# ksil/LFPSQP.jl

Hardware: AMD Instinct MI355X
Metric: projected-CG iters/sec at n=1e7, m=128 fp64 (higher is better)
Workload: dtype f64

## Files before the change

### include/lfpsqp_hip.h

```cpp
#ifndef LFPSQP_HIP_H
#define LFPSQP_HIP_H

#include <stdint.h>

#ifdef __cplusplus
extern "C" {
#endif

#define LFPSQP_OK 0
#define LFPSQP_ERR_ARG (-1)
#define LFPSQP_ERR_HIP (-2)
#define LFPSQP_ERR_COMM (-3)
#define LFPSQP_ERR_NUMERIC (-4)
#define LFPSQP_ERR_UNSUPPORTED (-5)

typedef struct lfpsqp_ctx lfpsqp_ctx;
typedef struct lfpsqp_vec lfpsqp_vec;
typedef struct lfpsqp_mat lfpsqp_mat;
typedef struct lfpsqp_spmat lfpsqp_spmat;

int lfpsqp_ctx_create(int device, lfpsqp_ctx** out);
int lfpsqp_ctx_destroy(lfpsqp_ctx* ctx);
int lfpsqp_ctx_sync(lfpsqp_ctx* ctx);
const char* lfpsqp_last_error(const lfpsqp_ctx* ctx);
int lfpsqp_device_name(const lfpsqp_ctx* ctx, char* buf, int64_t buflen);
int lfpsqp_device_uuid(const lfpsqp_ctx* ctx, char* buf, int64_t buflen);
int lfpsqp_ctx_set_tuning(lfpsqp_ctx* ctx, int ks, int nt);
int lfpsqp_ctx_set_onepass(lfpsqp_ctx* ctx, int mode);
int lfpsqp_ctx_set_residual_buffers(lfpsqp_ctx* ctx, int mode);
int lfpsqp_timer_begin(lfpsqp_ctx* ctx);
int lfpsqp_timer_end(lfpsqp_ctx* ctx, double* ms);

int lfpsqp_shard_range(int64_t n, int rank, int nranks, int64_t* row0, int64_t* row1);
int lfpsqp_comm_unique_id(lfpsqp_ctx* ctx, void* id128);
int lfpsqp_comm_init_rccl(lfpsqp_ctx* ctx, int rank, int nranks, const void* id128);
typedef int (*lfpsqp_allreduce_fn)(void* user, double* buf, int64_t count, int op, void* stream);
int lfpsqp_comm_init_callback(lfpsqp_ctx* ctx, int rank, int nranks, lfpsqp_allreduce_fn fn, void* user);
int lfpsqp_comm_p2p_export(lfpsqp_ctx* ctx, void* handle64);
int lfpsqp_comm_init_p2p(lfpsqp_ctx* ctx, int rank, int nranks, const void* handles);
#define LFPSQP_P2P_MEM_NONE 0
#define LFPSQP_P2P_MEM_FINE 1
#define LFPSQP_P2P_MEM_COARSE 2
int lfpsqp_comm_p2p_allow_coarse(lfpsqp_ctx* ctx, int allow);
int lfpsqp_comm_p2p_info(const lfpsqp_ctx* ctx, int* mem_kind, unsigned long long* collectives);
int lfpsqp_comm_info(const lfpsqp_ctx* ctx, int* rank, int* nranks);

int lfpsqp_vec_alloc(lfpsqp_ctx* ctx, int64_t n, lfpsqp_vec** out);
int lfpsqp_vec_free(lfpsqp_ctx* ctx, lfpsqp_vec* v);
int64_t lfpsqp_vec_len(const lfpsqp_vec* v);
int lfpsqp_vec_upload(lfpsqp_ctx* ctx, lfpsqp_vec* v, int64_t offset, const double* host, int64_t count);
int lfpsqp_vec_download(lfpsqp_ctx* ctx, const lfpsqp_vec* v, int64_t offset, double* host, int64_t count);
int lfpsqp_vec_fill(lfpsqp_ctx* ctx, lfpsqp_vec* v, double value);
int lfpsqp_vec_copy(lfpsqp_ctx* ctx, lfpsqp_vec* dst, const lfpsqp_vec* src);
int lfpsqp_vec_copy_range(lfpsqp_ctx* ctx, lfpsqp_vec* dst, int64_t dst_off, const lfpsqp_vec* src, int64_t src_off, int64_t count);
int lfpsqp_mat_alloc(lfpsqp_ctx* ctx, int64_t n, int64_t m, lfpsqp_mat** out);
int lfpsqp_mat_free(lfpsqp_ctx* ctx, lfpsqp_mat* M);
int lfpsqp_mat_shape(const lfpsqp_mat* M, int64_t* n, int64_t* m);
int lfpsqp_mat_upload(lfpsqp_ctx* ctx, lfpsqp_mat* M, int64_t col0, int64_t ncols, const double* host, int64_t ldh);
int lfpsqp_mat_download(lfpsqp_ctx* ctx, const lfpsqp_mat* M, int64_t col0, int64_t ncols, double* host, int64_t ldh);
int lfpsqp_mat_copy(lfpsqp_ctx* ctx, lfpsqp_mat* dst, const lfpsqp_mat* src);
int lfpsqp_mat_view(lfpsqp_ctx* ctx, const lfpsqp_mat* A, const lfpsqp_vec* rs, const lfpsqp_vec* u, const lfpsqp_vec* w, lfpsqp_mat** out);
int lfpsqp_mat_rowscaled_view(lfpsqp_ctx* ctx, const lfpsqp_mat* A, const lfpsqp_vec* rs, lfpsqp_mat** out);
int lfpsqp_ctx_set_placement(lfpsqp_ctx* ctx, int tries);
int lfpsqp_mat_alloc_placed(lfpsqp_ctx* ctx, int64_t n, int64_t m, lfpsqp_mat** out);
int lfpsqp_vecs_alloc_placed(lfpsqp_ctx* ctx, const lfpsqp_mat* M, int64_t ncols, int64_t n, int count, lfpsqp_vec** out);
int lfpsqp_basis_work_alloc_placed(lfpsqp_ctx* ctx, int64_t n, int64_t m, int64_t nvec, int count, lfpsqp_mat** M_out, lfpsqp_vec** out);
int lfpsqp_placement_info(const lfpsqp_ctx* ctx, int* tries, int* picked, double* ms, int ms_cap);
int lfpsqp_placement_probe(lfpsqp_ctx* ctx, const lfpsqp_mat* M, int64_t ncols, lfpsqp_vec* g, lfpsqp_vec* d, lfpsqp_vec* a, int reps, double* ms);
int lfpsqp_vec_hash_fill(lfpsqp_ctx* ctx, lfpsqp_vec* v, uint64_t seed, int64_t offset, double scale, double shift);
int lfpsqp_mat_hash_fill(lfpsqp_ctx* ctx, lfpsqp_mat* M, uint64_t seed, int64_t row0, int64_t n_global, double scale, int64_t nrows,
                         int64_t ncols);

int lfpsqp_gemv_t(lfpsqp_ctx* ctx, const lfpsqp_mat* M, int64_t ncols, const lfpsqp_vec* v, lfpsqp_vec* t);
int lfpsqp_gemv_n(lfpsqp_ctx* ctx, const lfpsqp_mat* M, int64_t ncols, double alpha, const lfpsqp_vec* t, double beta, lfpsqp_vec* y);
int lfpsqp_dot(lfpsqp_ctx* ctx, const lfpsqp_vec* x, const lfpsqp_vec* y, double* out);
int lfpsqp_dot_head(lfpsqp_ctx* ctx, const lfpsqp_vec* x, const lfpsqp_vec* y, int64_t count, double* out);
int lfpsqp_nrm2(lfpsqp_ctx* ctx, const lfpsqp_vec* x, double* out);
int lfpsqp_amax(lfpsqp_ctx* ctx, const lfpsqp_vec* x, double* out);
int lfpsqp_axpby(lfpsqp_ctx* ctx, double a, const lfpsqp_vec* x, double b, lfpsqp_vec* y);
int lfpsqp_waxpby(lfpsqp_ctx* ctx, double a, const lfpsqp_vec* x, double b, const lfpsqp_vec* y, lfpsqp_vec* z);
int lfpsqp_vmul(lfpsqp_ctx* ctx, const lfpsqp_vec* d, const lfpsqp_vec* x, lfpsqp_vec* y);
int lfpsqp_vec_fill_range(lfpsqp_ctx* ctx, lfpsqp_vec* v, int64_t offset, int64_t count, double value);
// ... 231 lines not shown
```

### lfpsqp.jl_amd/_capi.py

```python
from __future__ import annotations

import ctypes as C
import os
import re

_HERE = os.path.dirname(os.path.abspath(__file__))
DEFAULT_LIB = os.path.join(_HERE, "lib", "liblfpsqp_hip.so")
HEADER = os.path.join(os.path.dirname(_HERE), "include", "lfpsqp_hip.h")

c_i64 = C.c_int64
c_dbl = C.c_double
P = C.c_void_p
PD = C.POINTER(C.c_double)


class DiagOp(C.Structure):
    _fields_ = [("a0", c_dbl), ("dg", P)]


class LowRankOp(C.Structure):
    _fields_ = [("a0", c_dbl), ("dg", P), ("V", P), ("k", c_i64), ("sigma", P)]


class TridiagOp(C.Structure):
    _fields_ = [("a0", c_dbl), ("dg", P), ("off", P)]


class Basis(C.Structure):
    _fields_ = [("Z", P), ("ncols", c_i64), ("Dx", P), ("Dy", P), ("sx", P), ("sy", P), ("A", P), ("W", P), ("S", P), ("SA", P)]


class IneqData(C.Structure):
    _fields_ = [("q", P), ("r", P), ("s", P), ("t", P), ("n", c_i64)]


class Elementwise(C.Structure):
    _fields_ = [("A", P), ("Asp", P), ("kind", P), ("qw", P), ("work", P)]


class Constraints(C.Structure):
    _fields_ = [("Jct", P), ("m_lin", c_i64), ("b", P), ("has_ball", C.c_int), ("R2", c_dbl), ("n_x", c_i64), ("slack_row", c_i64), ("Jsp", P),
                ("ew", C.POINTER(Elementwise))]


CFUN = C.CFUNCTYPE(C.c_int, P, P, PD)
JACFUN = C.CFUNCTYPE(C.c_int, P, P, P, PD)


class PPWork(C.Structure):
    _fields_ = [(k, P) for k in ("r", "p", "z", "dx", "g", "tmp_m", "tmp_w", "h", "DxS", "DyS", "ones", "zeros", "q", "i11", "i12", "i22")] + \
               [("precondition", C.c_int)]


class PcgPrecond(C.Structure):
    _fields_ = [("K", P), ("i11", P), ("i12", P), ("i22", P), ("q", P)]


class ProjCGWorkC(C.Structure):
    _fields_ = [("g", P), ("d", P), ("rp", P), ("Utr", P)]


ALLREDUCE_FN = C.CFUNCTYPE(C.c_int, P, P, c_i64, C.c_int, P)
OPFUN = C.CFUNCTYPE(C.c_int, P, P, P)

_SIGS = {
    "lfpsqp_ctx_create": [C.c_int, C.POINTER(P)],
    "lfpsqp_ctx_destroy": [P],
    "lfpsqp_ctx_sync": [P],
    "lfpsqp_ctx_set_tuning": [P, C.c_int, C.c_int],
    "lfpsqp_ctx_set_onepass": [P, C.c_int],
    "lfpsqp_factored_basis_supported": [P, P, P, C.POINTER(C.c_int)],
    "lfpsqp_ctx_set_residual_buffers": [P, C.c_int],
    "lfpsqp_device_name": [P, C.c_char_p, c_i64],
    "lfpsqp_device_uuid": [P, C.c_char_p, c_i64],
    "lfpsqp_timer_begin": [P],
    "lfpsqp_timer_end": [P, PD],
    "lfpsqp_shard_range": [c_i64, C.c_int, C.c_int, C.POINTER(c_i64), C.POINTER(c_i64)],
    "lfpsqp_comm_unique_id": [P, P],
    "lfpsqp_comm_init_rccl": [P, C.c_int, C.c_int, P],
    "lfpsqp_comm_init_callback": [P, C.c_int, C.c_int, ALLREDUCE_FN, P],
    "lfpsqp_comm_p2p_export": [P, P],
    "lfpsqp_comm_init_p2p": [P, C.c_int, C.c_int, P],
    "lfpsqp_comm_p2p_allow_coarse": [P, C.c_int],
    "lfpsqp_comm_p2p_info": [P, C.POINTER(C.c_int), C.POINTER(C.c_ulonglong)],
    "lfpsqp_comm_info": [P, C.POINTER(C.c_int), C.POINTER(C.c_int)],
    "lfpsqp_vec_alloc": [P, c_i64, C.POINTER(P)],
    "lfpsqp_vec_free": [P, P],
    "lfpsqp_vec_upload": [P, P, c_i64, P, c_i64],
    "lfpsqp_vec_download": [P, P, c_i64, P, c_i64],
    "lfpsqp_vec_fill": [P, P, c_dbl],
    "lfpsqp_vec_copy": [P, P, P],
    "lfpsqp_vec_copy_range": [P, P, c_i64, P, c_i64, c_i64],
    "lfpsqp_mat_alloc": [P, c_i64, c_i64, C.POINTER(P)],
    "lfpsqp_mat_free": [P, P],
    "lfpsqp_ctx_set_placement": [P, C.c_int],
    "lfpsqp_ctx_set_nr_batch_mode": [P, C.c_int],
    "lfpsqp_mat_alloc_placed": [P, c_i64, c_i64, C.POINTER(P)],
    "lfpsqp_vecs_alloc_placed": [P, P, c_i64, c_i64, C.c_int, C.POINTER(P)],
    "lfpsqp_basis_work_alloc_placed": [P, c_i64, c_i64, c_i64, C.c_int, C.POINTER(P), C.POINTER(P)],
    "lfpsqp_placement_info": [P, C.POINTER(C.c_int), C.POINTER(C.c_int), PD, C.c_int],
    "lfpsqp_placement_probe": [P, P, c_i64, P, P, P, C.c_int, PD],
    "lfpsqp_mat_shape": [P, C.POINTER(c_i64), C.POINTER(c_i64)],
    "lfpsqp_mat_upload": [P, P, c_i64, c_i64, P, c_i64],
    "lfpsqp_mat_download": [P, P, c_i64, c_i64, P, c_i64],
    "lfpsqp_mat_copy": [P, P, P],
    "lfpsqp_mat_rowscaled_view": [P, P, P, C.POINTER(P)],
    "lfpsqp_mat_view": [P, P, P, P, P, C.POINTER(P)],
    "lfpsqp_factorize_hint": [P, P, c_i64],
    "lfpsqp_vec_hash_fill": [P, P, C.c_uint64, c_i64, c_dbl, c_dbl],
    "lfpsqp_mat_hash_fill": [P, P, C.c_uint64, c_i64, c_i64, c_dbl, c_i64, c_i64],
    "lfpsqp_gemv_t": [P, P, c_i64, P, P],
    "lfpsqp_gemv_n": [P, P, c_i64, c_dbl, P, c_dbl, P],
    "lfpsqp_dot": [P, P, P, PD],
    "lfpsqp_dot_head": [P, P, P, c_i64, PD],
    "lfpsqp_nrm2": [P, P, PD],
    "lfpsqp_amax": [P, P, PD],
    "lfpsqp_axpby": [P, c_dbl, P, c_dbl, P],
    "lfpsqp_waxpby": [P, c_dbl, P, c_dbl, P, P],
    "lfpsqp_vmul": [P, P, P, P],
    "lfpsqp_vec_fill_range": [P, P, c_i64, c_i64, c_dbl],
    "lfpsqp_affine_head": [P, c_dbl, P, c_dbl, c_i64, P],
    "lfpsqp_sumsq_shift": [P, P, c_i64, c_dbl, PD],
    "lfpsqp_allreduce": [P, P, c_i64],
    "lfpsqp_ineq_data_build": [P, P, P, P, P, P, P],
    "lfpsqp_generate_initial_y": [P, P, C.POINTER(IneqData)],
# ... 120 lines not shown
```

### lfpsqp.jl_amd/csrc/context.hip

```cpp
#include <dlfcn.h>
#include <stdarg.h>
#include <stdio.h>
#include <stdlib.h>
#include <ctype.h>
#include <string.h>

#include <algorithm>

#include "internal.h"

namespace lfpsqp {

int set_err(lfpsqp_ctx* ctx, int code, const char* fmt, ...) {
    char buf[1024];
    va_list ap;
    va_start(ap, fmt);
    vsnprintf(buf, sizeof(buf), fmt, ap);
    va_end(ap);
    if (ctx) ctx->err = buf;
    else fprintf(stderr, "lfpsqp: %s\n", buf);
    return code;
}

static int regrow(lfpsqp_ctx* ctx, double** buf, size_t* have, size_t cap, bool zero) {
// ... 220 lines not shown
inline hipError_t dev_alloc(void** out, size_t bytes) { return hipMalloc(out, bytes); }
inline void dev_free(void* p) { (void)hipFree(p); }
}

__global__ __launch_bounds__(lfpsqp::kThreads) void view_copy_kernel(const double* __restrict__ A, const double* __restrict__ rs, const double* __restrict__ u,
                                                                     const double* __restrict__ w, double* __restrict__ D, int64_t ld, int64_t n, int m) {
    const int64_t i = ((int64_t)blockIdx.x * lfpsqp::kThreads + threadIdx.x) * 2;
    if (i >= n) return;
    const double2 s = rs ? lfpsqp::ld2(rs + i) : make_double2(1.0, 1.0);
    const double2 uu = u ? lfpsqp::ld2(u + i) : make_double2(0.0, 0.0);
    const bool v1 = i + 1 < n;
    const int j0 = blockIdx.y * 16, j1 = (j0 + 16 < m) ? j0 + 16 : m;
#pragma unroll 4
    for (int j = j0; j < j1; ++j) {
        const double2 c = lfpsqp::ld2(A + (int64_t)j * ld + i);
        const double wj = u ? w[j] : 0.0;
        const double2 o = make_double2(fma(uu.x, wj, s.x * c.x), fma(uu.y, wj, s.y * c.y));
        if (v1) lfpsqp::st2(D + (int64_t)j * ld + i, o);
        else D[(int64_t)j * ld + i] = o.x;
    }
}

extern "C" {

int lfpsqp_ctx_create(int device, lfpsqp_ctx** out) {
    if (!out) return LFPSQP_ERR_ARG;
    *out = nullptr;
    int ndev = 0;
    if (hipGetDeviceCount(&ndev) != hipSuccess || ndev <= 0) return set_err(nullptr, LFPSQP_ERR_HIP, "no HIP device visible");
    if (device < 0 || device >= ndev) return set_err(nullptr, LFPSQP_ERR_ARG, "device %d out of range (%d visible)", device, ndev);
    lfpsqp_ctx* ctx = new lfpsqp_ctx();
    ctx->device = device;
    if (hipSetDevice(device) != hipSuccess) { delete ctx; return set_err(nullptr, LFPSQP_ERR_HIP, "hipSetDevice(%d) failed", device); }
    hipDeviceProp_t prop;
    if (hipGetDeviceProperties(&prop, device) == hipSuccess) {
        ctx->devname = std::string(prop.name) + " (" + prop.gcnArchName + ")";
        ctx->num_cu = prop.multiProcessorCount;
        ctx->real_gpu = strncmp(prop.gcnArchName, "gfx", 3) == 0;
    }
    bool ok = hipStreamCreate(&ctx->stream) == hipSuccess;
    ok = ok && hipMalloc((void**)&ctx->scal, 64 * sizeof(double)) == hipSuccess;
    ok = ok && hipMalloc((void**)&ctx->istat, 128 * sizeof(int64_t)) == hipSuccess;
    ok = ok && hipHostMalloc((void**)&ctx->h_scal, 4 * 64 * sizeof(double)) == hipSuccess;
    ok = ok && hipHostMalloc((void**)&ctx->h_istat, 4 * 16 * sizeof(int64_t)) == hipSuccess;
    for (int i = 0; ok && i < 4; ++i) ok = hipEventCreate(&ctx->ev_slot[i]) == hipSuccess;
    ok = ok && hipEventCreate(&ctx->ev_t0) == hipSuccess && hipEventCreate(&ctx->ev_t1) == hipSuccess;
    if (ok) ok = hipMemset(ctx->scal, 0, 64 * sizeof(double)) == hipSuccess && hipMemset(ctx->istat, 0, 128 * sizeof(int64_t)) == hipSuccess;
    if (!ok) { delete ctx; return set_err(nullptr, LFPSQP_ERR_HIP, "context resource allocation failed"); }
    if (const char* e = getenv("LFPSQP_ONEPASS")) ctx->tune_onepass = atoi(e);
    if (const char* e = getenv("LFPSQP_SPGRAM")) ctx->tune_spgram = atoi(e) < 0 ? -1 : 0;
    if (const char* e = getenv("LFPSQP_VEC_BLOCKS")) ctx->tune_vec_blocks = atoi(e) > 0 ? atoi(e) : 0;
    if (const char* e = getenv("LFPSQP_NRB_MFMA")) ctx->tune_nrb_mfma = atoi(e) > 0 ? 1 : (atoi(e) < 0 ? -1 : 0);
    if (const char* e = getenv("LFPSQP_GPING")) ctx->tune_gping = atoi(e) == 1 ? 1 : 0;
    if (const char* e = getenv("LFPSQP_NRB_WG_CAP")) ctx->batch_wg_cap = atoi(e) > 0 ? atoi(e) : 0;
    if (const char* e = getenv("LFPSQP_STAGE_ROUNDS")) ctx->stage_cap = atoi(e) > 0 ? atoi(e) : 0;
    *out = ctx;
    return 0;
}

int lfpsqp_ctx_destroy(lfpsqp_ctx* ctx) {
    if (!ctx) return 0;
    (void)hipSetDevice(ctx->device);
    (void)hipStreamSynchronize(ctx->stream);
    if (ctx->comm.kind == Comm::RCCL && ctx->comm.nccl_comm && ctx->comm.ncclCommDestroy) ctx->comm.ncclCommDestroy(ctx->comm.nccl_comm);
    for (int r = 0; r < kP2PMaxRanks; ++r)
        if (ctx->comm.p2p_peer[r] && ctx->comm.p2p_peer[r] != ctx->comm.p2p_mine) (void)hipIpcCloseMemHandle(ctx->comm.p2p_peer[r]);
    if (ctx->comm.p2p_mine) (void)hipFree(ctx->comm.p2p_mine);
    if (ctx->comm.p2p_err) (void)hipHostFree(ctx->comm.p2p_err);
    if (ctx->prof_init)
        for (int s = 0; s < kProfSlots; ++s)
            for (int e = 0; e < kProfEvents; ++e)
                for (int k = 0; k < 2; ++k) (void)hipEventDestroy(ctx->prof_ev[s][e][k]);
    for (int i = 0; i < 4; ++i) if (ctx->ev_slot[i]) (void)hipEventDestroy(ctx->ev_slot[i]);
    if (ctx->ev_t0) (void)hipEventDestroy(ctx->ev_t0);
    if (ctx->ev_t1) (void)hipEventDestroy(ctx->ev_t1);
    if (ctx->part) (void)hipFree(ctx->part);
    if (ctx->small) (void)hipFree(ctx->small);
    if (ctx->d_m) (void)hipFree(ctx->d_m);
    if (ctx->d_qw) (void)hipFree(ctx->d_qw);
    if (ctx->d_zeros) (void)hipFree(ctx->d_zeros);
    if (ctx->d_nvec) (void)hipFree(ctx->d_nvec);
    if (ctx->d_tri) (void)hipFree(ctx->d_tri);
    if (ctx->d_view) (void)hipFree(ctx->d_view);
    if (ctx->h_m) (void)hipHostFree(ctx->h_m);
    if (ctx->scal) (void)hipFree(ctx->scal);
    if (ctx->istat) (void)hipFree(ctx->istat);
    if (ctx->h_scal) (void)hipHostFree(ctx->h_scal);
    if (ctx->h_istat) (void)hipHostFree(ctx->h_istat);
    if (ctx->stream) (void)hipStreamDestroy(ctx->stream);
    delete ctx;
    return 0;
}

int lfpsqp_ctx_sync(lfpsqp_ctx* ctx) {
    LF_ARG(ctx, ctx != nullptr);
    LF_HIP(ctx, hipStreamSynchronize(ctx->stream));
    return 0;
}

const char* lfpsqp_last_error(const lfpsqp_ctx* ctx) { return ctx ? ctx->err.c_str() : "null context"; }

int lfpsqp_device_name(const lfpsqp_ctx* ctx, char* buf, int64_t buflen) {
    if (!ctx || !buf || buflen <= 0) return LFPSQP_ERR_ARG;
    snprintf(buf, (size_t)buflen, "%s", ctx->devname.c_str());
    return 0;
}
// ... 4 lines not shown
    memset(&id, 0, sizeof(id));
    hipDevice_t d;
    if (hipDeviceGet(&d, ctx->device) != hipSuccess || hipDeviceGetUuid(&id, d) != hipSuccess) {
        (void)hipGetLastError();
        snprintf(buf, (size_t)buflen, "unknown");
        return 0;
    }
    bool hexchars = true;
    for (int i = 0; i < 16; ++i) hexchars = hexchars && isxdigit((unsigned char)id.bytes[i]);
    int o = snprintf(buf, (size_t)buflen, "GPU-");
    for (int i = 0; i < 16; ++i)
        o += hexchars ? snprintf(buf + o, (size_t)buflen - o, "%c", id.bytes[i]) : snprintf(buf + o, (size_t)buflen - o, "%02x", (unsigned char)id.bytes[i]);
    return 0;
}

int lfpsqp_timer_begin(lfpsqp_ctx* ctx) {
    LF_ARG(ctx, ctx != nullptr);
    LF_HIP(ctx, hipEventRecord(ctx->ev_t0, ctx->stream));
    return 0;
}
int lfpsqp_timer_end(lfpsqp_ctx* ctx, double* ms) {
    LF_ARG(ctx, ctx != nullptr && ms != nullptr);
    LF_HIP(ctx, hipEventRecord(ctx->ev_t1, ctx->stream));
    LF_HIP(ctx, hipEventSynchronize(ctx->ev_t1));
    float f = 0.f;
    LF_HIP(ctx, hipEventElapsedTime(&f, ctx->ev_t0, ctx->ev_t1));
    *ms = f;
    return 0;
}

int lfpsqp_ctx_set_tuning(lfpsqp_ctx* ctx, int ks, int nt) {
    LF_ARG(ctx, ctx != nullptr && (ks == 0 || ks == 2 || ks == 4));
    LF_HIP(ctx, hipStreamSynchronize(ctx->stream));
    ctx->tune_ks = ks;
    ctx->tune_nt = nt != 0;
    return 0;
}

int lfpsqp_ctx_set_onepass(lfpsqp_ctx* ctx, int mode) {
    LF_ARG(ctx, ctx != nullptr && (mode == 0 || mode == -1));
    LF_HIP(ctx, hipStreamSynchronize(ctx->stream));
    ctx->tune_onepass = mode;
    return 0;
}

int lfpsqp_ctx_set_residual_buffers(lfpsqp_ctx* ctx, int mode) {
    LF_ARG(ctx, ctx != nullptr && (mode == 0 || mode == 1));
    LF_HIP(ctx, hipStreamSynchronize(ctx->stream));
    ctx->tune_gping = mode;
    ctx->pcg_resume.valid = false;
    return 0;
}

int lfpsqp_ctx_set_profiling(lfpsqp_ctx* ctx, int on) {
    LF_ARG(ctx, ctx != nullptr);
    if (on && prof_lazy_init(ctx) != 0) return set_err(ctx, LFPSQP_ERR_HIP, "profiling event creation failed");
    ctx->profiling = on != 0;
    for (int s = 0; s < kProfSlots; ++s) { ctx->prof_used[s] = 0; ctx->prof_count[s] = 0; ctx->prof_ms[s] = 0.0; ctx->prof_seq[s] = 0; ctx->prof_live[s] = false; }
    return 0;
}
int lfpsqp_profile_read(lfpsqp_ctx* ctx, double ms[8], int64_t counts[8]) {
    LF_ARG(ctx, ctx != nullptr && ms && counts);
    LF_HIP(ctx, hipStreamSynchronize(ctx->stream));
    prof_collect(ctx);
    for (int s = 0; s < kProfSlots; ++s) { ms[s] = ctx->prof_ms[s]; counts[s] = ctx->prof_count[s]; }
    return 0;
}


int lfpsqp_shard_range(int64_t n, int rank, int nranks, int64_t* row0, int64_t* row1) {
    if (n < 0 || nranks <= 0 || rank < 0 || rank >= nranks || !row0 || !row1) return LFPSQP_ERR_ARG;
    const int64_t tiles = (n + kPadRows - 1) / kPadRows;
    const int64_t base = tiles / nranks, extra = tiles % nranks;
    const int64_t t0 = (int64_t)rank * base + (rank < extra ? rank : extra);
    const int64_t t1 = t0 + base + (rank < extra ? 1 : 0);
    int64_t r0 = t0 * kPadRows, r1 = t1 * kPadRows;
    if (r0 > n) r0 = n;
    if (r1 > n) r1 = n;
    *row0 = r0;
    *row1 = r1;
    return 0;
}

static int load_rccl(lfpsqp_ctx* ctx) {
    Comm& c = ctx->comm;
    if (c.rccl_lib) return 0;
    const char* names[] = {"librccl.so.1", "librccl.so", "/opt/rocm/lib/librccl.so.1"};
    for (const char* nm : names) {
        c.rccl_lib = dlopen(nm, RTLD_NOW | RTLD_LOCAL);
        if (c.rccl_lib) break;
    }
    if (!c.rccl_lib) return set_err(ctx, LFPSQP_ERR_COMM, "cannot dlopen librccl: %s", dlerror());
    return 0;
}

int lfpsqp_comm_unique_id(lfpsqp_ctx* ctx, void* id128) {
    LF_ARG(ctx, ctx != nullptr && id128 != nullptr);
    LF_TRY(load_rccl(ctx));
    typedef int (*get_id_fn)(void*);
    get_id_fn f = (get_id_fn)dlsym(ctx->comm.rccl_lib, "ncclGetUniqueId");
    if (!f) return set_err(ctx, LFPSQP_ERR_COMM, "ncclGetUniqueId not found");
    int rc = f(id128);
    if (rc != 0) return set_err(ctx, LFPSQP_ERR_COMM, "ncclGetUniqueId failed (%d)", rc);
    return 0;
}

// ... 480 lines not shown
```

### lfpsqp.jl_amd/csrc/internal.h

```cpp
#pragma once
#include <hip/hip_runtime.h>
#include <stdint.h>

#include <string>
#include <vector>

#include "../../include/lfpsqp_hip.h"
#include "kernels.h"

struct lfpsqp_slab {
    void* p = nullptr;
    int refs = 0;
};
struct lfpsqp_vec {
    double* p = nullptr;
    int64_t n = 0;
    int64_t cap = 0;
    lfpsqp_slab* slab = nullptr;
};

constexpr int64_t kLdSkewDefault = 16;

struct lfpsqp_mat {
    double* p = nullptr;
// ... 22 lines not shown
    bool p2p_allow_coarse = false;
    void* rccl_lib = nullptr;
    void* nccl_comm = nullptr;
    int (*ncclAllReduce)(const void*, void*, size_t, int , int , void*, hipStream_t) = nullptr;
    int (*ncclCommDestroy)(void*) = nullptr;
    const char* (*ncclGetErrorString)(int) = nullptr;
    lfpsqp_allreduce_fn cb = nullptr;
    void* cb_user = nullptr;
};

}

struct lfpsqp_ctx {
    int device = 0;
    int num_cu = 0;
    hipStream_t stream = nullptr;
    std::string err;
    std::string devname;
    lfpsqp::Comm comm;
    bool comm_active() const { return comm.kind != lfpsqp::Comm::NONE; }

    double* part = nullptr;
    size_t part_cap = 0;
    double* small = nullptr;
    size_t small_cap = 0;
    double* d_m = nullptr;
    double* h_m = nullptr;
    size_t m_cap = 0;
    std::vector<double> warm_V;
    int warm_m = 0;
    double* d_view = nullptr;
    double* d_nvec = nullptr;
    size_t nvec_cap = 0;
    double* d_tri = nullptr;
    size_t tri_cap = 0;
    double* d_zeros = nullptr;
    double* d_qw = nullptr;
    size_t qw_cap = 0;
    double* scal = nullptr;
    int64_t* istat = nullptr;
    double* h_scal = nullptr;
    int64_t* h_istat = nullptr;
    hipEvent_t ev_slot[4] = {nullptr, nullptr, nullptr, nullptr};
    hipEvent_t ev_t0 = nullptr, ev_t1 = nullptr;

    int tune_ks = 0;
    bool tune_nt = true;
    int ks_for(int64_t n) const { return tune_ks ? tune_ks : (n >= 4000000 ? 4 : 2); }
    int tune_onepass = 0;
    int tune_spgram = 0;
    int tune_vec_blocks = 0;
    int tune_nrb_mfma = -1;
    int tune_gping = 0;

    bool real_gpu = false;
    int place_tries = 3;
    int64_t place_min_bytes = (int64_t)1 << 30;
    double place_last_ms[64] = {0};
    int place_last_n = 0, place_last_pick = 0;

    struct ProjcgResume {
        bool valid = false;
        const double *x = nullptr, *g = nullptr, *d = nullptr, *Z = nullptr;
        int m = 0;
        int64_t nv = 0, iters = 0;
        bool gcur_is_rp = false;
        const double *dg = nullptr, *b = nullptr;
        double a0 = 0.0;
        int64_t n_global = 0;
        uint64_t epoch = 0;
    } pcg_resume;
    int batch_wg_cap = 0;
    int stage_cap = 0;
    uint64_t launch_epoch = 0;

    bool profiling = false;
    hipEvent_t prof_ev[lfpsqp::kProfSlots][lfpsqp::kProfEvents][2];
    int prof_used[lfpsqp::kProfSlots] = {0};
    int64_t prof_seq[lfpsqp::kProfSlots] = {0};
    bool prof_live[lfpsqp::kProfSlots] = {false};
    int64_t prof_count[lfpsqp::kProfSlots] = {0};
    double prof_ms[lfpsqp::kProfSlots] = {0};
    bool prof_init = false;
};

namespace lfpsqp {

int set_err(lfpsqp_ctx* ctx, int code, const char* fmt, ...);
int ensure_part(lfpsqp_ctx* ctx, size_t doubles);
int ensure_small(lfpsqp_ctx* ctx, size_t doubles);
int ensure_tri(lfpsqp_ctx* ctx, size_t doubles);
int ensure_mvec(lfpsqp_ctx* ctx, size_t doubles);
int ensure_nvec(lfpsqp_ctx* ctx, size_t doubles);

struct Layout {
    struct Region { double** p; size_t at; };
    Region r[12];
    int k = 0;
    size_t n = 0;
    size_t skip(size_t len, size_t align = 2) {
        const size_t at = (n + align - 1) / align * align;
        n = at + len;
        return at;
    }
    void add(double*& p, size_t len, size_t align = 2) { r[k++] = Region{&p, skip(len, align)}; }
    size_t size() const { return n; }
// ... 396 lines not shown
```

### lfpsqp.jl_amd/csrc/projcg.hip

```cpp
#include <math.h>
#include <stdlib.h>

#include <algorithm>
#include <vector>

#include "internal.h"
#include "sparse.h"
#include "sphess.h"

namespace lfpsqp {

enum { S_DAD = 0, S_RG = 1, S_ALPHA = 2, S_RPGP = 3, S_GPGP = 4, S_BETA = 5, S_NR = 6, S_TOL = 7, S_DD = 8, S_ALPHA_PREV = 9 };
enum { I_STATUS = 0, I_ITER = 1, I_MAXIT = 2 };
enum { ST_RUNNING = 0, ST_CONVERGED = 1, ST_RG_BREAK = 2, ST_NEGCURV = 3, ST_MAXIT = 4 };

struct AOpD {
    double a0;
    const double* dg;
    __device__ __forceinline__ double2 apply(int64_t i, double2 d) const {
        if (dg) {
            const double2 q = ld2(dg + i);
            return make_double2((a0 + q.x) * d.x, (a0 + q.y) * d.y);
        }
        return make_double2(a0 * d.x, a0 * d.y);
// ... 927 lines not shown
            dAd_next = fma(beta * beta, dAd, fma(-2.0 * beta, gAd, gAg));
        }
        if (st == ST_RUNNING) {
            u.istat[I_ITER] = it + 1;
            u.scal[S_DAD] = dAd_next;
            if (dAd_next <= 0.0) st = ST_NEGCURV;
            else if (gpgp <= 0.0) st = ST_RG_BREAK;
            else {
                u.scal[S_ALPHA_PREV] = (u.init == 2) ? 0.0 : ld_scal(u.scal + S_ALPHA);
                u.scal[S_ALPHA] = gpgp / dAd_next;
            }
            if (st != ST_RUNNING) u.hm.publish(st, it + 1, nr);
        }
        if (st != ST_RUNNING) u.istat[I_STATUS] = st;
        go = (st == ST_RUNNING);
        sh[0] = gpgp / dAd_next;
        sh[1] = beta;
        if (go)
            for (int j = 0; j < u.k; ++j) {
                const double vg = ld_scal(S + 5 + j);
                const double vd = (u.init == 1) ? -vg : fma(beta, u.vdraw[j], -vg);
                u.vdraw[j] = vd;
                u.vdc[j] = ld_scal(u.sigma + j) * vd;
            }
    }
    __syncthreads();
    if (!go) return;
    const double alpha = sh[0], beta = sh[1];
    for (int j = threadIdx.x; j < u.m; j += blockDim.x) {
        const double t1 = ld_scal(u.T + j);
        double t2 = ld_scal(u.T + u.m + j);
        if (u.triM) t2 -= s_mu[j];
        for (int l = 0; l < u.k; ++l)
            t2 = fma(u.UtV[(size_t)l * u.m + j], ld_scal(u.sigma + l) * ld_scal(u.T + 2 * u.m + 5 + l), t2);
        const double t3 = (u.init == 1) ? -t2 : fma(beta, u.t3[j], -t2);
        u.t3[j] = t3;
        const double ut = fma(alpha, t3, t1);
        u.Utr[j] = ut;
        if (u.W) s_utr[j] = ut;
    }
    if (u.W) {
        __syncthreads();
        const double* const xin[1] = {nullptr};
        double yo[1];
        small_wdot<1>(u.W, 1, (size_t)u.wm, u.wm, u.m, xin, s_utr, yo, s_part);
        int rp = 32;
        while (rp < u.wm) rp <<= 1;
        if ((int)threadIdx.x < u.wm && (int)threadIdx.x / rp == 0) u.uA[threadIdx.x] = yo[0];
    }
}
#ifndef LFPSQP_K1_NT
#define LFPSQP_K1_NT 1
#endif
struct PcgDirG {
    double* d;
    const double* g;
    double* x;
    const double* scal;
    const int64_t* istat;
    int force;
    __device__ __forceinline__ bool skip() const { return !force && ld_stat(istat + I_STATUS) != ST_RUNNING; }
    __device__ __forceinline__ void apply(int64_t i, bool v0, bool v1, double*) const {
        double2 dd = ld2(d + i);
        if (!force) {
            const double alpha = ld_scal(scal + S_ALPHA_PREV);
            double2 xx = ld2(x + i);
            xx = make_double2(fma(alpha, dd.x, xx.x), fma(alpha, dd.y, xx.y));
            if (v1) { if (LFPSQP_K1_NT >= 1) st2_stream(x + i, xx); else st2(x + i, xx); }
            else if (v0) x[i] = xx.x;
        }
        const double beta = ld_scal(scal + S_BETA);
        const double2 gg = ld2(g + i);
        dd = make_double2(beta * dd.x - gg.x, beta * dd.y - gg.y);
        if (v1) { if (LFPSQP_K1_NT == 1) st2_stream(d + i, dd); else st2(d + i, dd); }
        else if (v0) d[i] = dd.x;
    }
};

template <class AOP>
struct ResidualV {
    const double* x;
    const double* b;
    double* out;
    AOP A;
    double sgn;
    __device__ __forceinline__ bool skip() const { return false; }
    __device__ __forceinline__ double2 load(int64_t r, bool v0, bool v1) const {
        const double2 xx = ld2(x + r), bb = ld2(b + r);
        const double2 ax = A.apply(r, xx);
        const double2 rr = make_double2(sgn * (ax.x - bb.x), sgn * (ax.y - bb.y));
        if (out) {
            if (v1) st2(out + r, rr);
            else if (v0) out[r] = rr.x;
        }
        return make_double2(v0 ? rr.x : 0.0, v1 ? rr.y : 0.0);
    }
};
struct InitState {
    double* scal;
    int64_t* istat;
    double tol;
    int64_t maxit;
    __device__ __forceinline__ bool skip() const { return false; }
    __device__ __forceinline__ void run(double*) const {
        for (int k = 0; k < 16; ++k) scal[k] = 0.0;
        scal[S_TOL] = tol;
        scal[S_NR] = INFINITY;
        istat[I_STATUS] = ST_RUNNING;
        istat[I_ITER] = 0;
        istat[I_MAXIT] = maxit;
    }
};
struct FlushXF {
    double* x;
    const double* d;
    const double* scal;
    __device__ __forceinline__ bool skip() const { return false; }
    __device__ __forceinline__ void apply(int64_t i, bool v0, bool v1, double*) const {
        const double alpha = ld_scal(scal + S_ALPHA);
        const double2 dd = ld2(d + i);
        double2 xx = ld2(x + i);
        xx = make_double2(fma(alpha, dd.x, xx.x), fma(alpha, dd.y, xx.y));
        if (v1) st2(x + i, xx);
        else if (v0) x[i] = xx.x;
    }
};
// ... 539 lines not shown
    const AOpV Aop{(callback || cop) ? Av->p : nullptr};
    auto residual_with = [&](auto aop, double sgn, double* store, double* t_out) -> int {
        using AOP = decltype(aop);
        const ResidualV<AOP> rv{x->p, b->p, store, aop, sgn};
        if (SA && stacked) return sp_gemv_t(ResidualVS<AOP>{rv, sk, store ? nullptr : lambda->p}, tmpN, t_out, store ? uA : nullptr);
        if (DF && stacked) return df_gemv_t(ResidualVS<AOP>{rv, sk, store ? nullptr : lambda->p}, t_out, store ? uDF : nullptr);
        if (DF) return df_gemv_t(rv, t_out, store ? uDF : nullptr);
        if (stacked) return run_gemv_t(ctx, Z, m, N, ResidualVS<AOP>{rv, sk, store ? nullptr : lambda->p}, t_out);
        if (SA) return sp_gemv_t(rv, tmpN, t_out, store ? uA : nullptr);
        return run_gemv_t(ctx, Z, m, N, rv, t_out);
    };
    auto launch_residual = [&](double sgn, double* store, double* t_out) -> int {
        if (kLR > 0) {
            LF_TRY(run_gemv_t(ctx, LRop->V, kLR, N, SpPlainV{x->p}, lrVtv));
            return residual_with(AOpLR{Ad.a0, Ad.dg, LRop->V->p, LRop->V->ld, kLR, lrSig, lrVtv}, sgn, store, t_out);
        }
        if (cop) {
            LF_TRY(coupled_mul(ctx, *cop, nv, N, x->p, Av->p));
            return residual_with(Aop, sgn, store, t_out);
        }
        if (!callback) return residual_with(Ad, sgn, store, t_out);
        LF_TRY(apply_op(x));
        return residual_with(Aop, sgn, store, t_out);
    };
    auto k2_with = [&](auto aop) -> int {
        using AOP = decltype(aop);
        const PcgStepV<AOP> sv{d, g, aop, scal, istat};
        if (SA && stacked) return sp_gemv_t(PcgStepVS<AOP>{sv, sk}, tmpN, Utr, uA);
        if (stacked) return run_gemv_t(ctx, Z, m, N, PcgStepVS<AOP>{sv, sk}, Utr, 1);
        if (SA) return sp_gemv_t(sv, tmpN, Utr, uA);
        return run_gemv_t(ctx, Z, m, N, sv, Utr, 1);
    };
    auto launch_k2 = [&]() -> int { return callback ? k2_with(Aop) : k2_with(Ad); };
    auto k3_with = [&](auto aop, int init) -> int {
        using AOP = decltype(aop);
        const PcgProjE<AOP> pe{rp, g, d, istat, init, PcgStepV<AOP>{d, g, aop, scal, istat}};
        const PcgPost3 post{scal, istat, init, hm, scal + S_RPGP};
        if (SA && stacked) {
            using E = PcgProjES<AOP>;
            const SpConsumeE<E> ce{E{pe, sk}, ell_rows(SA, uA), U->A->p + (int64_t)SA->m * U->A->ld, U->A->ld, uA + SA->m, nxs};
            return run_vec<SpConsumeE<E>, 2, PcgPost3>(ctx, N, ce, 0u, scal + S_RPGP, post, init ? -1 : 2);
        }
        if (stacked) return run_gemv_n<PcgProjES<AOP>, 2, PcgPost3>(ctx, Z, m, N, Utr, PcgProjES<AOP>{pe, sk}, scal + S_RPGP, post, init ? -1 : 2);
        if (SA) {
            using E = PcgProjE<AOP>;
            const SpConsumeE<E> ce{pe, ell_rows(SA, uA), U->A->p + (int64_t)SA->m * U->A->ld, U->A->ld, uA + SA->m, nxs};
            return run_vec<SpConsumeE<E>, 2, PcgPost3>(ctx, nv, ce, 0u, scal + S_RPGP, post, init ? -1 : 2);
        }
        return run_gemv_n<PcgProjE<AOP>, 2, PcgPost3>(ctx, Z, m, N, Utr, pe, scal + S_RPGP, post, init ? -1 : 2);
    };
    auto launch_k3 = [&](int init) -> int { return callback ? k3_with(Aop, init) : k3_with(Ad, init); };

    const bool kPing = ctx->tune_gping == 1;
    double* gbuf[2] = {g, (fused && kPing && !cop) ? rp : g};
    int gcur = 0;
    auto prepare_neighbours = [&](auto STc, auto INc, const double* src, const double* dsrc, double* ad, double* q) -> int {
        constexpr bool ST = decltype(STc)::value, INIT = decltype(INc)::value;
        if (cop->kind == CoupledOp::BAND)
            return with_band(cop->K, [&](auto Bc) -> int {
                constexpr int B = decltype(Bc)::value;
                const BandD<B> Ab = cop->template band<B>(N, N);
                if constexpr (ST) return run_vec<TriPrepSF<B, INIT>, 0, NoPost>(ctx, N, TriPrepSF<B, INIT>{Ab, hs, sk.Dx, sk.Dy, src, dsrc, ad, q, scal, istat}, 0u, nullptr, NoPost());
                else return run_vec<TriPrepF<B, INIT>, 0, NoPost>(ctx, N, TriPrepF<B, INIT>{Ab, src, dsrc, ad, q, scal, istat}, 0u, nullptr, NoPost());
            });
        return with_gathers(*cop, N, N, [&](auto Ab) -> int {
            using D = decltype(Ab);
            if constexpr (ST) {
                double* ux = tri_ux(ctx);
                LF_TRY((run_vec<DiagsPrepSF<D, INIT>, 0, NoPost>(ctx, N, DiagsPrepSF<D, INIT>{Ab, hs, sk.Dx, sk.Dy, src, dsrc, ad, ux, scal, istat}, 0u, nullptr, NoPost())));
                return run_vec<DiagsGatherF<D>, 0, NoPost>(ctx, N, DiagsGatherF<D>{Ab, ux, nullptr, q, scal, istat}, 0u, nullptr, NoPost());
            } else {
                if constexpr (!INIT) LF_TRY((run_vec<DiagsMulF<D>, 0, NoPost>(ctx, N, DiagsMulF<D>{Ab, dsrc, ad, istat}, 0u, nullptr, NoPost())));
                return run_vec<DiagsGatherF<D>, 0, NoPost>(ctx, N, DiagsGatherF<D>{Ab, src, ad, q, scal, istat}, 0u, nullptr, NoPost());
            }
        });
    };
    auto launch_fused = [&](int init) -> int {
        const int slot = init ? -1 : 3;
        const double* gin = gbuf[gcur];
        double* gout = init ? gbuf[0] : gbuf[gcur ^ 1];
        const double* tin = DF ? uDF : Utr;
        double* Tout = DF ? Traw : T12;
        auto fuse_lr = [&](auto INc) -> int {
            constexpr bool INIT = decltype(INc)::value;
            return run_onepass<PcgFuseLR<INIT>, 2, 5 + kLRMax>(ctx, Z, mc, mc, N, tin, PcgFuseLR<INIT>{rp, gin, gout, d, Ad, scal, istat, LRop->V->p, LRop->V->ld, kLR, lrVdc}, Tout, slot);
        };
        if (cop) LF_TRY(with_stacked_init(stacked, init != 0, [&](auto STc, auto INc) -> int {
            constexpr bool ST = decltype(STc)::value, INIT = decltype(INc)::value;
            const double* src = INIT ? rp : gin;
            const double* dsrc = INIT ? nullptr : d;
            double* ad = INIT ? nullptr : Av->p;
            double* q = INIT ? Av->p : rp;
            LF_TRY(prepare_neighbours(STc, INc, src, dsrc, ad, q));
            return run_onepass<PcgFuseTri<ST, INIT>, 2, 5>(ctx, Z, mc, mc, N, tin, PcgFuseTri<ST, INIT>{rp, gin, gout, d, ad, q, Ad, scal, istat, sk}, Tout, slot);
        }));
        else if (kLR > 0) LF_TRY(init ? fuse_lr(std::true_type{}) : fuse_lr(std::false_type{}));
        else LF_TRY(with_stacked_init(stacked, init != 0, [&](auto STc, auto INc) -> int {
            constexpr bool ST = decltype(STc)::value, INIT = decltype(INc)::value;
            return run_onepass<PcgFuseE<ST, INIT>, 2, 5>(ctx, Z, mc, mc, N, tin, PcgFuseE<ST, INIT>{rp, gin, gout, d, Ad, scal, istat, sk}, Tout, slot);
        }));
        if (!init) gcur ^= 1;
        PcgPostF pf{T12, t3, Utr, scal, istat, m, init, hm, dWf, Traw, T12, uDF, DF ? mc : 0};
        if (kLR > 0) { pf.k = kLR; pf.UtV = lrUtV; pf.sigma = lrSig; pf.vdraw = lrVdraw; pf.vdc = lrVdc; }
        pf.triM = dTriM;
        hipLaunchKernelGGL(pcg_post_kernel, dim3(1), dim3(DF ? 1024 : 256), 0, ctx->stream, pf);
        LF_LAUNCH_CHECK(ctx);
// ... 15 lines not shown
        const int64_t lim = maxit_eff;
        LF_HIP(ctx, hipMemcpyAsync(istat + I_MAXIT, &lim, sizeof(int64_t), hipMemcpyHostToDevice, ctx->stream));
        LF_HIP(ctx, hipStreamSynchronize(ctx->stream));
        hipLaunchKernelGGL(pcg_post_kernel, dim3(1), dim3(DF ? 1024 : 256), 0, ctx->stream, PcgPostF{T12, t3, Utr, scal, istat, m, 2, hm, dWf, Traw, T12, uDF, DF ? mc : 0});
        LF_LAUNCH_CHECK(ctx);
    }
    ctx->pcg_resume.valid = false;
    if (!resume) {
        hipLaunchKernelGGL((post_kernel<InitState>), dim3(1), dim3(1), 0, ctx->stream, scal, InitState{scal, istat, tol, maxit_eff});
        LF_LAUNCH_CHECK(ctx);

        if (c && m > 0) {
            if (!DF) LF_TRY(lfpsqp_gemv_n(ctx, Z, m, 1.0, c, 0.0, x));
        } else {
            LF_TRY(lfpsqp_vec_fill(ctx, x, 0.0));
        }
        if (kLR > 0) {
            for (int j = 0; j < kLRMax; ++j) ctx->h_m[j] = (j < kLR) ? (LRop->sigma ? LRop->sigma[j] : 1.0) : 0.0;
            LF_HIP(ctx, hipMemcpyAsync(lrSig, ctx->h_m, sizeof(double) * kLRMax, hipMemcpyHostToDevice, ctx->stream));
            LF_HIP(ctx, hipStreamSynchronize(ctx->stream));
            LF_HIP(ctx, hipMemsetAsync(lrVdraw, 0, sizeof(double) * 3 * kLRMax, ctx->stream));
            for (int l = 0; l < kLR; ++l) {
                const SpPlainV col{LRop->V->p + (int64_t)l * LRop->V->ld};
                if (DF) LF_TRY(df_gemv_t(col, lrUtV + (size_t)l * m, nullptr));
                else LF_TRY(run_gemv_t(ctx, Z, m, N, col, lrUtV + (size_t)l * m));
            }
        }
        if (flags & LFPSQP_PROJCG_START_PROJECTED) {
            if (!(DF && fused && !c && kLR == 0) || work->Utr->n < (int64_t)mc + 2 * m + 5)
                return set_err(ctx, LFPSQP_ERR_UNSUPPORTED, "LFPSQP_PROJCG_START_PROJECTED: basis in factored form over a dense generator, c == NULL, work->Utr of >= A.m + 2 ncols + 5 entries");
            LF_HIP(ctx, hipMemcpyAsync(T12, Utr + mc, sizeof(double) * (2 * (size_t)m + 5), hipMemcpyDeviceToDevice, ctx->stream));
            PcgPostF pf{T12, t3, Utr, scal, istat, m, 1, hm, dWf, Traw, T12, uDF, mc};
            pf.pre = 1;
            hipLaunchKernelGGL(pcg_post_kernel, dim3(1), dim3(1024), 0, ctx->stream, pf);
            LF_LAUNCH_CHECK(ctx);
        } else if (flags & LFPSQP_PROJCG_START_GIVEN) {
            if (!(DF && fused && !c))
                return set_err(ctx, LFPSQP_ERR_UNSUPPORTED, "LFPSQP_PROJCG_START_GIVEN: basis in factored form over a dense generator, c == NULL");
            LF_TRY(factored_w_times_t(ctx, dWf, mc, m, Utr, uDF));
        } else {
            LF_TRY(launch_residual(1.0, rp, Utr));
        }
        if (flags & LFPSQP_PROJCG_START_PROJECTED) {  }
        else if (fused) LF_TRY(launch_fused(1));
        else LF_TRY(launch_k3(1));
    }

    int64_t it = 0;
    bool done = false;
    const int gcur_start = gcur;
    const int64_t it_end = maxit_eff - it_base;
    while (!done && it < it_end) {
        if (fused) {
            if (it > 0 || resume) LF_TRY((run_vec<PcgDirG, 0, NoPost>(ctx, nv, PcgDirG{d, gbuf[gcur], x->p, scal, istat, 0}, 0u, nullptr, NoPost(), 0)));
            LF_TRY(launch_fused(0));
        } else if (callback) {
            if (it > 0) LF_TRY((run_vec<PcgDirX, 0, NoPost>(ctx, nv, PcgDirX{d, g, x->p, scal, istat}, 0u, nullptr, NoPost(), 0)));
            LF_TRY(apply_op(work->d));
            LF_TRY((run_vec<DotPairF, 1, PcgPost1>(ctx, nv, DotPairF{d, Av->p, istat}, 0u, scal + S_DAD, PcgPost1{scal, istat, hm})));
            LF_TRY(launch_k2());
            LF_TRY(launch_k3(0));
        } else {
            LF_TRY((run_vec<PcgDirF, 1, PcgPost1>(ctx, nv, PcgDirF{d, g, x->p, Ad, scal, istat, it == 0 ? 1 : 0}, 0u, scal + S_DAD,
                                                  PcgPost1{scal, istat, hm}, 0)));
            LF_TRY(launch_k2());
            LF_TRY(launch_k3(0));
        }
        LF_HIP(ctx, hipEventRecord(ctx->ev_slot[it & 3], ctx->stream));
        if (it >= 2) {
            LF_HIP(ctx, hipEventSynchronize(ctx->ev_slot[(it - 2) & 3]));
            if (hstat[kRingOff + ((it_base + it - 1) % kRing)] != ST_RUNNING) done = true;
        }
        ++it;
    }
    LF_HIP(ctx, hipStreamSynchronize(ctx->stream));
    const int64_t status = hstat[0];
    *iters = hstat[1];
    *nr = *(volatile double*)ctx->h_scal;
    if (fused) {
        const int64_t executed = ((status == ST_CONVERGED || status == ST_MAXIT) ? *iters : *iters - 1) - it_base;
        gcur = (gbuf[1] != gbuf[0]) ? (int)((gcur_start + (executed > 0 ? executed : 0)) & 1) : 0;
    }

    if ((status == ST_CONVERGED || status == ST_MAXIT || (fused && status == ST_RG_BREAK && *iters > 1)) && *iters > it_base)
        LF_TRY((run_vec<FlushXF, 0, NoPost>(ctx, nv, FlushXF{x->p, d, scal}, 0u, nullptr, NoPost())));
    if (fused && status == ST_MAXIT && *iters > 0 && kLR == 0 && !cop)
        ctx->pcg_resume = lfpsqp_ctx::ProjcgResume{true, x->p, g, d, Z->p, m, nv, *iters, gcur == 1, Ad.dg, b->p, Ad.a0, n_global, ctx->launch_epoch};
    if (status == ST_NEGCURV) {
        if (fused && *iters > 1)
            LF_TRY((run_vec<PcgDirG, 0, NoPost>(ctx, nv, PcgDirG{d, gbuf[gcur], x->p, scal, istat, 1}, 0u, nullptr, NoPost())));
        LF_TRY((run_vec<SumSqF, 1, NoPost>(ctx, nv, SumSqF{d}, 0u, scal + S_DD, NoPost())));
        LF_TRY((run_vec<NormalizeIntoF, 0, NoPost>(ctx, nv, NormalizeIntoF{x->p, d, scal + S_DD}, 0u, nullptr, NoPost())));
        if (lambda) LF_TRY(lfpsqp_vec_fill(ctx, lambda, NAN));
        *nr = INFINITY;
    } else if (flags & LFPSQP_PROJCG_WANT_LAMBDA) {
        if (stacked) LF_TRY(launch_residual(-1.0, nullptr, lambda->p + N));
        else if (m > 0) LF_TRY(launch_residual(-1.0, nullptr, lambda->p));
    }
    if (ctx->profiling) {
        LF_HIP(ctx, hipStreamSynchronize(ctx->stream));
        prof_collect(ctx);
    }
    return 0;
}

int lfpsqp::placement_probe(lfpsqp_ctx* ctx, const lfpsqp_mat* M, int ncols, double* g, double* d, double* a, int reps, double* ms) {
    *ms = -1.0;
    if (!M || M->n <= 0 || ncols < 4 || ncols > M->m || onepass_cw(ctx, ncols, M->ld, M->n) == 0) return 0;
    double *T12, *Utr;
    Layout L;
    L.add(T12, 2 * ncols + 5); L.add(Utr, ncols); L.skip(18);
    LF_TRY(ensure_mvec(ctx, L.size()));
    L.carve(ctx->d_m);
    LF_HIP(ctx, hipMemsetAsync(ctx->d_m, 0, sizeof(double) * L.size(), ctx->stream));
    hipLaunchKernelGGL((post_kernel<InitState>), dim3(1), dim3(1), 0, ctx->stream, ctx->scal, InitState{ctx->scal, ctx->istat, 0.0, (int64_t)1 << 40});
    LF_LAUNCH_CHECK(ctx);
    const StackD sk{0, nullptr, nullptr, nullptr, nullptr};
    const Comm::Kind saved = ctx->comm.kind;
    ctx->comm.kind = Comm::NONE;
    int rc = 0;
    for (int k = 0; k < reps + 1 && rc == 0; ++k) {
        if (k == 1) rc = hipEventRecord(ctx->ev_t0, ctx->stream) == hipSuccess ? 0 : LFPSQP_ERR_HIP;
        if (rc == 0) rc = with_stacked_init(false, false, [&](auto STc, auto INc) -> int {
            constexpr bool ST = decltype(STc)::value, INIT = decltype(INc)::value;
            return run_onepass<PcgFuseE<ST, INIT>, 2, 5>(ctx, M, ncols, ncols, M->n, Utr, PcgFuseE<ST, INIT>{g, g, g, d, AOpD{0.0, a}, ctx->scal, ctx->istat, sk}, T12, -1);
        });
    }
    ctx->comm.kind = saved;
    LF_TRY(rc);
    LF_HIP(ctx, hipEventRecord(ctx->ev_t1, ctx->stream));
    LF_HIP(ctx, hipEventSynchronize(ctx->ev_t1));
    float t = 0.f;
    LF_HIP(ctx, hipEventElapsedTime(&t, ctx->ev_t0, ctx->ev_t1));
    *ms = (double)t / reps;
    return 0;
}

// ... 142 lines not shown
```

### lfpsqp.jl_amd/device.py

```python
from __future__ import annotations

import ctypes as C

import numpy as np

from . import _capi
from ._capi import LfpsqpError, P, c_i64


class Context:

    def __init__(self, device: int = 0, lib: _capi.Library | None = None):
        self.L = lib or _capi.load_library()
        h = P()
        rc = self.L.lfpsqp_ctx_create(device, C.byref(h))
        if rc != 0 or not h:
            raise LfpsqpError(f"lfpsqp_ctx_create(device={device}) failed (status {rc}): no usable MI355X/HIP device; "
                              "the product path has no CPU fallback")
        self.h = h
        self.rank, self.nranks = 0, 1
        self._cb_keep = None
        from .params import DeviceOptions
        self.options = DeviceOptions()

    def check(self, rc: int):
        if rc != 0:
            raise LfpsqpError(f"status {rc}: {self.L.lfpsqp_last_error(self.h).decode()}")

    def close(self):
        if getattr(self, "h", None):
            self.L.lfpsqp_ctx_destroy(self.h)
            self.h = None

    def sync(self):
        self.check(self.L.lfpsqp_ctx_sync(self.h))

    @property
    def device_name(self) -> str:
        buf = C.create_string_buffer(256)
        self.check(self.L.lfpsqp_device_name(self.h, buf, 256))
        return buf.value.decode()

    def device_uuid(self) -> str:
        buf = C.create_string_buffer(64)
        self.check(self.L.lfpsqp_device_uuid(self.h, buf, 64))
        return buf.value.decode()

    def timer_begin(self):
        self.check(self.L.lfpsqp_timer_begin(self.h))

    def timer_end(self) -> float:
        ms = C.c_double()
        self.check(self.L.lfpsqp_timer_end(self.h, C.byref(ms)))
        return ms.value

    def factored_basis_supported(self, A, SA=None) -> bool:
        yes = C.c_int(0)
        self.check(self.L.lfpsqp_factored_basis_supported(self.h, A.h, SA.h if SA is not None else None, C.byref(yes)))
        return bool(yes.value)

    def set_onepass(self, mode: int = 0):
        self.check(self.L.lfpsqp_ctx_set_onepass(self.h, int(mode)))

    def set_residual_buffers(self, mode: int = 0):
        self.check(self.L.lfpsqp_ctx_set_residual_buffers(self.h, int(mode)))

    def set_placement(self, tries: int = 3):
        self.check(self.L.lfpsqp_ctx_set_placement(self.h, int(tries)))
        self.options.placement_tries = int(tries)

    def set_nr_batch_mode(self, matrix_cores: bool = False):
        self.check(self.L.lfpsqp_ctx_set_nr_batch_mode(self.h, 1 if matrix_cores else 0))
        self.options.ls_batch_matrix_cores = bool(matrix_cores)

    def free_memory(self):
        try:
            import ctypes.util
            hip = C.CDLL("libamdhip64.so")
            f, t = C.c_size_t(), C.c_size_t()
            if hip.hipMemGetInfo(C.byref(f), C.byref(t)) == 0:
                return int(f.value)
        except OSError:
            pass
        return None

    def placement_info(self):
        tries, pick = C.c_int(), C.c_int()
        ms = (C.c_double * 64)()
        self.check(self.L.lfpsqp_placement_info(self.h, C.byref(tries), C.byref(pick), ms, 64))
        return tries.value, pick.value, list(ms)[:tries.value]

    def _wrap_vecs(self, hh, n, count, stacked_N, hs):
        out = []
        for k in range(count):
            if stacked_N is not None:
                from .inequality import StackedVector
                v = StackedVector.__new__(StackedVector)
                v.N, v.hs = int(stacked_N), hs
            else:
                v = DeviceVector.__new__(DeviceVector)
            v.ctx, v.n, v.h = self, int(n), P(hh[k])
            out.append(v)
        return out

    def basis_and_vectors_placed(self, n: int, m: int, count: int, stacked_N: int | None = None):
        hs, nv = None, int(n)
        if stacked_N is not None:
            hs = int(self.L.lfpsqp_half_stride(int(stacked_N)))
            nv = hs + int(stacked_N)
        hh = (P * count)()
        mh = P()
        self.check(self.L.lfpsqp_basis_work_alloc_placed(self.h, int(n), int(m), nv, int(count), C.byref(mh), hh))
        M = DeviceMatrix.__new__(DeviceMatrix)
        M.ctx, M.n, M.m, M.h = self, int(n), int(m), mh
        return M, self._wrap_vecs(hh, nv, count, stacked_N, hs)

    def vectors_placed(self, M: "DeviceMatrix | None", n: int, count: int, ncols: int | None = None, stacked_N: int | None = None):
        hs = None
# ... 318 lines not shown
```

Measured before the change: 584.6.

## Pair x updates across two CG iterations and halve host event syncs

The fused direction kernel now updates x only on every other iteration, applying both the previous alpha*d and the current alpha*d_new in one read-modify-write. This roughly halves x traffic per iteration. Host-side event recording and synchronization now run every two iterations in fused mode, which reduces host overhead but may detect termination one iteration later. The final flush of x is skipped when the pairing has already applied the last update, so correctness at termination boundaries depends on this parity bookkeeping.

```diff
diff --git a/include/lfpsqp_hip.h b/include/lfpsqp_hip.h
--- a/include/lfpsqp_hip.h
+++ b/include/lfpsqp_hip.h
@@ -28,6 +28,7 @@
 int lfpsqp_ctx_set_tuning(lfpsqp_ctx* ctx, int ks, int nt);
 int lfpsqp_ctx_set_onepass(lfpsqp_ctx* ctx, int mode);
 int lfpsqp_ctx_set_residual_buffers(lfpsqp_ctx* ctx, int mode);
+int lfpsqp_ctx_set_x_pairing(lfpsqp_ctx* ctx, int mode);
 int lfpsqp_timer_begin(lfpsqp_ctx* ctx);
 int lfpsqp_timer_end(lfpsqp_ctx* ctx, double* ms);
 
diff --git a/lfpsqp.jl_amd/_capi.py b/lfpsqp.jl_amd/_capi.py
--- a/lfpsqp.jl_amd/_capi.py
+++ b/lfpsqp.jl_amd/_capi.py
@@ -71,6 +71,7 @@
     "lfpsqp_ctx_set_onepass": [P, C.c_int],
     "lfpsqp_factored_basis_supported": [P, P, P, C.POINTER(C.c_int)],
     "lfpsqp_ctx_set_residual_buffers": [P, C.c_int],
+    "lfpsqp_ctx_set_x_pairing": [P, C.c_int],
     "lfpsqp_device_name": [P, C.c_char_p, c_i64],
     "lfpsqp_device_uuid": [P, C.c_char_p, c_i64],
     "lfpsqp_timer_begin": [P],
diff --git a/lfpsqp.jl_amd/csrc/context.hip b/lfpsqp.jl_amd/csrc/context.hip
--- a/lfpsqp.jl_amd/csrc/context.hip
+++ b/lfpsqp.jl_amd/csrc/context.hip
@@ -296,6 +296,7 @@
     if (const char* e = getenv("LFPSQP_VEC_BLOCKS")) ctx->tune_vec_blocks = atoi(e) > 0 ? atoi(e) : 0;
     if (const char* e = getenv("LFPSQP_NRB_MFMA")) ctx->tune_nrb_mfma = atoi(e) > 0 ? 1 : (atoi(e) < 0 ? -1 : 0);
     if (const char* e = getenv("LFPSQP_GPING")) ctx->tune_gping = atoi(e) == 1 ? 1 : 0;
+    if (const char* e = getenv("LFPSQP_X_PAIR")) ctx->tune_xpair = atoi(e) == 0 ? 0 : 1;
     if (const char* e = getenv("LFPSQP_NRB_WG_CAP")) ctx->batch_wg_cap = atoi(e) > 0 ? atoi(e) : 0;
     if (const char* e = getenv("LFPSQP_STAGE_ROUNDS")) ctx->stage_cap = atoi(e) > 0 ? atoi(e) : 0;
     *out = ctx;
@@ -406,6 +407,13 @@
     return 0;
 }
 
+int lfpsqp_ctx_set_x_pairing(lfpsqp_ctx* ctx, int mode) {
+    LF_ARG(ctx, ctx != nullptr && (mode == 0 || mode == 1));
+    LF_HIP(ctx, hipStreamSynchronize(ctx->stream));
+    ctx->tune_xpair = mode;
+    return 0;
+}
+
 int lfpsqp_ctx_set_profiling(lfpsqp_ctx* ctx, int on) {
     LF_ARG(ctx, ctx != nullptr);
     if (on && prof_lazy_init(ctx) != 0) return set_err(ctx, LFPSQP_ERR_HIP, "profiling event creation failed");
diff --git a/lfpsqp.jl_amd/csrc/internal.h b/lfpsqp.jl_amd/csrc/internal.h
--- a/lfpsqp.jl_amd/csrc/internal.h
+++ b/lfpsqp.jl_amd/csrc/internal.h
@@ -98,6 +98,7 @@
     int tune_vec_blocks = 0;
     int tune_nrb_mfma = -1;
     int tune_gping = 0;
+    int tune_xpair = 1;
 
     bool real_gpu = false;
     int place_tries = 3;
diff --git a/lfpsqp.jl_amd/csrc/projcg.hip b/lfpsqp.jl_amd/csrc/projcg.hip
--- a/lfpsqp.jl_amd/csrc/projcg.hip
+++ b/lfpsqp.jl_amd/csrc/projcg.hip
@@ -1003,6 +1003,7 @@
 #ifndef LFPSQP_K1_NT
 #define LFPSQP_K1_NT 1
 #endif
+enum { K1_X_EACH = 0, K1_X_PAIR = 1, K1_X_NONE = 2 };
 struct PcgDirG {
     double* d;
     const double* g;
@@ -1010,19 +1011,28 @@
     const double* scal;
     const int64_t* istat;
     int force;
+    int xform = K1_X_EACH;
     __device__ __forceinline__ bool skip() const { return !force && ld_stat(istat + I_STATUS) != ST_RUNNING; }
     __device__ __forceinline__ void apply(int64_t i, bool v0, bool v1, double*) const {
         double2 dd = ld2(d + i);
-        if (!force) {
+        const bool with_x = !force && xform != K1_X_NONE;
+        double2 xx = make_double2(0.0, 0.0);
+        if (with_x) {
             const double alpha = ld_scal(scal + S_ALPHA_PREV);
-            double2 xx = ld2(x + i);
+            xx = ld2(x + i);
             xx = make_double2(fma(alpha, dd.x, xx.x), fma(alpha, dd.y, xx.y));
-            if (v1) { if (LFPSQP_K1_NT >= 1) st2_stream(x + i, xx); else st2(x + i, xx); }
-            else if (v0) x[i] = xx.x;
         }
         const double beta = ld_scal(scal + S_BETA);
         const double2 gg = ld2(g + i);
         dd = make_double2(beta * dd.x - gg.x, beta * dd.y - gg.y);
+        if (with_x) {
+            if (xform == K1_X_PAIR) {
+                const double alpha = ld_scal(scal + S_ALPHA);
+                xx = make_double2(fma(alpha, dd.x, xx.x), fma(alpha, dd.y, xx.y));
+            }
+            if (v1) { if (LFPSQP_K1_NT >= 1) st2_stream(x + i, xx); else st2(x + i, xx); }
+            else if (v0) x[i] = xx.x;
+        }
         if (v1) { if (LFPSQP_K1_NT == 1) st2_stream(d + i, dd); else st2(d + i, dd); }
         else if (v0) d[i] = dd.x;
     }
@@ -1668,6 +1678,7 @@
     auto launch_k3 = [&](int init) -> int { return callback ? k3_with(Aop, init) : k3_with(Ad, init); };
 
     const bool kPing = ctx->tune_gping == 1;
+    const bool xpair = ctx->tune_xpair == 1;
     double* gbuf[2] = {g, (fused && kPing && !cop) ? rp : g};
     int gcur = 0;
     auto prepare_neighbours = [&](auto STc, auto INc, const double* src, const double* dsrc, double* ad, double* q) -> int {
@@ -1789,7 +1800,8 @@
     const int64_t it_end = maxit_eff - it_base;
     while (!done && it < it_end) {
         if (fused) {
-            if (it > 0 || resume) LF_TRY((run_vec<PcgDirG, 0, NoPost>(ctx, nv, PcgDirG{d, gbuf[gcur], x->p, scal, istat, 0}, 0u, nullptr, NoPost(), 0)));
+            const int xform = !xpair ? K1_X_EACH : (((it_base + it + 1) & 1) == 0 ? K1_X_PAIR : K1_X_NONE);
+            if (it > 0 || resume) LF_TRY((run_vec<PcgDirG, 0, NoPost>(ctx, nv, PcgDirG{d, gbuf[gcur], x->p, scal, istat, 0, xform}, 0u, nullptr, NoPost(), 0)));
             LF_TRY(launch_fused(0));
         } else if (callback) {
             if (it > 0) LF_TRY((run_vec<PcgDirX, 0, NoPost>(ctx, nv, PcgDirX{d, g, x->p, scal, istat}, 0u, nullptr, NoPost(), 0)));
@@ -1803,10 +1815,14 @@
             LF_TRY(launch_k2());
             LF_TRY(launch_k3(0));
         }
-        LF_HIP(ctx, hipEventRecord(ctx->ev_slot[it & 3], ctx->stream));
-        if (it >= 2) {
-            LF_HIP(ctx, hipEventSynchronize(ctx->ev_slot[(it - 2) & 3]));
-            if (hstat[kRingOff + ((it_base + it - 1) % kRing)] != ST_RUNNING) done = true;
+        const int64_t stride = fused ? 2 : 1;
+        if ((it + 1) % stride == 0) {
+            LF_HIP(ctx, hipEventRecord(ctx->ev_slot[(it / stride) & 3], ctx->stream));
+            if (it >= 2) {
+                LF_HIP(ctx, hipEventSynchronize(ctx->ev_slot[((it - 2) / stride) & 3]));
+                for (int64_t q = 0; q < stride; ++q)
+                    if (hstat[kRingOff + ((it_base + it - 1 - q) % kRing)] != ST_RUNNING) done = true;
+            }
         }
         ++it;
     }
@@ -1819,7 +1835,9 @@
         gcur = (gbuf[1] != gbuf[0]) ? (int)((gcur_start + (executed > 0 ? executed : 0)) & 1) : 0;
     }
 
-    if ((status == ST_CONVERGED || status == ST_MAXIT || (fused && status == ST_RG_BREAK && *iters > 1)) && *iters > it_base)
+    const int64_t completed = (status == ST_CONVERGED || status == ST_MAXIT) ? *iters : *iters - 1;
+    const bool x_owed = !(fused && xpair) || (completed & 1) != 0;
+    if ((status == ST_CONVERGED || status == ST_MAXIT || (fused && status == ST_RG_BREAK)) && completed > it_base && x_owed)
         LF_TRY((run_vec<FlushXF, 0, NoPost>(ctx, nv, FlushXF{x->p, d, scal}, 0u, nullptr, NoPost())));
     if (fused && status == ST_MAXIT && *iters > 0 && kLR == 0 && !cop)
         ctx->pcg_resume = lfpsqp_ctx::ProjcgResume{true, x->p, g, d, Z->p, m, nv, *iters, gcur == 1, Ad.dg, b->p, Ad.a0, n_global, ctx->launch_epoch};
diff --git a/lfpsqp.jl_amd/device.py b/lfpsqp.jl_amd/device.py
--- a/lfpsqp.jl_amd/device.py
+++ b/lfpsqp.jl_amd/device.py
@@ -64,6 +64,9 @@
 
     def set_residual_buffers(self, mode: int = 0):
         self.check(self.L.lfpsqp_ctx_set_residual_buffers(self.h, int(mode)))
+
+    def set_x_pairing(self, mode: int = 1):
+        self.check(self.L.lfpsqp_ctx_set_x_pairing(self.h, int(mode)))
 
     def set_placement(self, tries: int = 3):
         self.check(self.L.lfpsqp_ctx_set_placement(self.h, int(tries)))
```

Result: faster. 594.2 (median of 6 runs) (+1.6%).
